# hungpham2511/toppra

Hardware: NVIDIA H100
Metric: paths/sec (7-DOF, 200 gridpoints, vel+accel) (higher is better)
Workload: dtype f64

## Files before the change

toppra_b200/csrc/tb_scan.cu:

```cuda
#include <limits.h>

#include "tb_common.cuh"
#include "tb_scan_common.cuh"

namespace tb {
namespace {

__device__ __forceinline__ uint32_t smem_u32(const void *p) { return (uint32_t)__cvta_generic_to_shared(p); }

__device__ __forceinline__ void mbar_init(uint64_t *bar, unsigned count) {
  asm volatile("mbarrier.init.shared::cta.b64 [%0], %1;" ::"r"(smem_u32(bar)), "r"(count) : "memory");
}
__device__ __forceinline__ void mbar_expect_tx_s(uint32_t bar, unsigned bytes) {
  asm volatile("mbarrier.arrive.expect_tx.shared::cta.b64 _, [%0], %1;" ::"r"(bar), "r"(bytes) : "memory");
}
__device__ __forceinline__ void bulk_g2s_s(uint32_t dst, const void *src, unsigned bytes, uint32_t bar) {
  asm volatile("cp.async.bulk.shared::cluster.global.mbarrier::complete_tx::bytes [%0], [%1], %2, [%3];" ::"r"(dst),
               "l"(src), "r"(bytes), "r"(bar)
               : "memory");
}
__device__ __forceinline__ void mbar_wait_s(const uint32_t addr, unsigned parity) {
  uint32_t ok;
  do {
    asm volatile(
        "{\n"
        " .reg .pred p;\n"
        " mbarrier.try_wait.parity.shared::cta.b64 p, [%1], %2;\n"
        " selp.u32 %0, 1, 0, p;\n"
        "}\n"
        : "=r"(ok)
        : "r"(addr), "r"(parity)
        : "memory");
    if (!ok) __nanosleep(64);
  } while (!ok);
}

__device__ __forceinline__ double warp_min(double v) {
  const int hi = __double2hiint(v), lo = __double2loint(v);
  const int m = hi >> 31;
  const unsigned khi = (unsigned)(hi ^ (m | (int)0x80000000)), klo = (unsigned)(lo ^ m);
  const unsigned mh = __reduce_min_sync(FULL, khi);
  const unsigned ml = __reduce_min_sync(FULL, khi == mh ? klo : 0xffffffffu);
  const int m2 = ((int)~mh) >> 31;
  return __hiloint2double((int)(mh ^ (unsigned)(m2 | (int)0x80000000)), (int)(ml ^ (unsigned)m2));
}
__device__ __forceinline__ double warp_max(double v) {
  const int hi = __double2hiint(v), lo = __double2loint(v);
  const int m = hi >> 31;
  const unsigned khi = (unsigned)(hi ^ (m | (int)0x80000000)), klo = (unsigned)(lo ^ m);
  const unsigned mh = __reduce_max_sync(FULL, khi);
  const unsigned ml = __reduce_max_sync(FULL, khi == mh ? klo : 0u);
  const int m2 = ((int)~mh) >> 31;
  return __hiloint2double((int)(mh ^ (unsigned)(m2 | (int)0x80000000)), (int)(ml ^ (unsigned)m2));
}

constexpr int SCAN_NBUF = 4;

__device__ __forceinline__ void project_item(const bool part, const double aj, const double bj, const double cj,
                                             const double dt0, const double dt1, const double z0, const double z1,
                                             double &thi, double &tlo, bool &bad) {
  const double denom = dt0 * aj + dt1 * bj;
  const double num = cj + z1 * bj + z0 * aj;
  const bool up = part && (denom > LP_TINY), dn = part && (denom < -LP_TINY);
  const double t = -num / ((up || dn) ? denom : 1.0);
  thi = (up && t < LP_INF) ? t : LP_INF;
  tlo = (dn && t > -LP_INF) ? t : -LP_INF;
  bad = bad || (part && !(up || dn) && (num > LP_SMALL));
}

__device__ __forceinline__ void box_row(const int m, const double low0, const double high0, const double low1,
                                        const double high1, double &aj, double &bj, double &cj) {
  aj = __hiloint2double((m == 0) ? (int)0xBFF00000 : ((m == 1) ? 0x3FF00000 : 0), 0);
  bj = __hiloint2double((m == 2) ? (int)0xBFF00000 : ((m == 3) ? 0x3FF00000 : 0), 0);
  cj = (m < 2) ? ((m == 0) ? low0 : -high0) : ((m == 2) ? low1 : -high1);
}

template <int RPL, bool PERM, bool SKIP>
__device__ __forceinline__ bool lp2d_impl(const double v0, const double v1, const double (&a)[RPL],
                                          const double (&b)[RPL], const double (&c)[RPL], const int nC,
                                          const double low0, const double high0, const double low1,
                                          const double high1, int &ac0, int &ac1, double &out_u, double &out_x,
                                          const int lane, int &n_resolve) {
  double p0 = (v0 > LP_TINY) ? high0 : low0;
  double p1 = (v1 > LP_TINY) ? high1 : low1;
  int nac0 = (v0 > LP_TINY) ? -2 : -1;
  int nac1 = (v1 > LP_TINY) ? -4 : -3;
  constexpr bool valid = PERM;
  int pos[RPL];
#pragma unroll
  for (int s = 0; s < RPL; ++s) {
    const int r = lane + 32 * s;
// ... 153 lines not shown
    if (__any_sync(FULL, bad || cross)) return false;
    if (tstar == (pick_min ? -LP_INF : LP_INF)) return false;
    int mykey = INT_MAX;
#pragma unroll
    for (int s = 0; s < RPL; ++s) mykey = ((pick_min ? tlo[s] : thi[s]) == tstar) ? min(mykey, key[s]) : mykey;
    if (!box_inline) mykey = ((pick_min ? xlo_t : xhi_t) == tstar) ? min(mykey, BOXBASE + lane) : mykey;
    const int akey = __reduce_min_sync(FULL, mykey);
    nac1 = (akey >= BOXBASE) ? (-1 - (akey - BOXBASE)) : pos_row(akey, valid, ac0, ac1);
    p0 = z0 + tstar * dt0;
    p1 = z1 + tstar * dt1;
  }
  ac0 = nac0;
  ac1 = nac1;
  out_u = p0;
  out_x = p1;
  return true;
}

template <int RPL, bool SKIP = false>
__device__ __forceinline__ bool lp2d_warp(const double v0, const double v1, const double (&a)[RPL],
                                          const double (&b)[RPL], const double (&c)[RPL], const int nC,
                                          const double low0, const double high0, const double low1,
                                          const double high1, int &ac0, int &ac1, double &out_u, double &out_x,
                                          const int lane, int &n_resolve) {
  if (low0 > high0 || low1 > high1) return false;
  const bool valid = ac0 >= 0 && ac0 < nC && ac1 >= 0 && ac1 < nC && ac0 != ac1;
  if (valid)
    return lp2d_impl<RPL, true, SKIP>(v0, v1, a, b, c, nC, low0, high0, low1, high1, ac0, ac1, out_u, out_x, lane,
                                       n_resolve);
  return lp2d_impl<RPL, false, SKIP>(v0, v1, a, b, c, nC, low0, high0, low1, high1, ac0, ac1, out_u, out_x, lane,
                                     n_resolve);
}

template <int RPL>
__device__ __forceinline__ bool lp1d_fixed_x_warp(const double v0, const double x, const double (&a)[RPL],
                                                  const double (&b)[RPL], const double (&c)[RPL],
                                                  const double low0, const double high0, double &out_u) {
  double my_hi = high0, my_lo = low0;
#pragma unroll
  for (int s = 0; s < RPL; ++s) {
    const double bxc = b[s] * x + c[s];
    const bool up = a[s] > LP_TINY, dn = a[s] < -LP_TINY;
    const double den = (up || dn) ? a[s] : 1.0;
    const bool zn = (bxc == 0.0);
    const double q = -opaque(zn ? 1.0 : bxc) / den;
    const double t = zn ? (-bxc) * den : q;
    my_hi = (up && t < my_hi) ? t : my_hi;
    my_lo = (dn && t > my_lo) ? t : my_lo;
  }
  const bool pick_min = (fabs(v0) < LP_TINY) || (v0 < 0);
  const double red = warp_min(pick_min ? -my_lo : my_hi);
  const double ustar = pick_min ? -red : red;
  if (__any_sync(FULL, pick_min ? (my_hi < ustar) : (my_lo > ustar))) return false;
  out_u = ustar;
  return true;
}

template <int RPL>
__device__ __forceinline__ void load_rows(const double *rec, const int R, const int nC, const int lane,
                                          double (&a)[RPL], double (&b)[RPL], double (&c)[RPL]) {
#pragma unroll
  for (int s = 0; s < RPL; ++s) {
    const int r = lane + 32 * s;
    const bool in = (r >= 2) && (r < nC);
    const int j = in ? r - 2 : 0;
    const double va = rec[j], vb = rec[R + j], vc = rec[2 * R + j];
    a[s] = in ? va : 0.0;
    b[s] = in ? vb : 0.0;
    c[s] = in ? vc : -1.0;
  }
}

template <int RPL>
__device__ __forceinline__ void set_xnext_rows(const int lane, const double delta, const double xn_min,
                                               const double xn_max, double (&a)[RPL], double (&b)[RPL],
                                               double (&c)[RPL]) {
  const bool xr = lane < 2, first = lane == 0;
  const double sgn = first ? -1.0 : 1.0;
  a[0] = xr ? sgn * (2 * delta) : a[0];
  b[0] = xr ? sgn : b[0];
  c[0] = xr ? (first ? xn_min : -xn_max) : c[0];
}

template <int RPL, int MINB, bool FAST, int CFLAGS = -1, bool FUSED = false, bool UB = false>
__global__ void __launch_bounds__(32, MINB)
scan_kernel(const double *__restrict__ records, const int W, const int R, const double *__restrict__ grid,
            const int grid_shared, const int B, const int G, const double *__restrict__ sd_start,
            const double *__restrict__ sd_end, const double *__restrict__ sd_end_hi, const int flags_arg,
            double *__restrict__ Kout, double *__restrict__ sdout, double *__restrict__ uout,
            int *__restrict__ status, int *__restrict__ fail_stage, int *__restrict__ counters,
            const int *__restrict__ glen, const VelAccSrc src) {
  static_assert(!FUSED || RPL == 1, "the fused row source holds one row per lane");
  static_assert(!(FUSED && UB), "velocity + acceleration problems have no u-bound");
  extern __shared__ __align__(16) unsigned char smem_raw[];
  int lane;
  asm volatile("mov.u32 %0, %%tid.x;" : "=r"(lane));
  const long path = blockIdx.x;
  if (path >= B) return;
  double *bufs = reinterpret_cast<double *>(smem_raw);
  uint64_t *bars = reinterpret_cast<uint64_t *>(smem_raw + (size_t)(FUSED ? 1 : SCAN_NBUF) * W * sizeof(double));
  const int Gp = (CFLAGS < 0 && glen) ? min(max(glen[path], 1), G) : G;
  const int N = Gp - 1, nC = R + 2;
  const unsigned rec_bytes = (unsigned)(W * sizeof(double));
  const void *volatile *sptr = reinterpret_cast<const void *volatile *>(
      smem_raw + (size_t)(FUSED ? 1 : SCAN_NBUF) * W * sizeof(double) + SCAN_NBUF * sizeof(uint64_t));
  if (lane == 0) {
    sptr[0] = FUSED ? static_cast<const void *>(src.xbound + (size_t)path * G * 2)
                    : static_cast<const void *>(records + (size_t)path * G * W);
    sptr[1] = grid + (grid_shared ? 0 : (size_t)path * G);
    sptr[2] = Kout + (size_t)path * G * 2;
  }
  const double *dco = bufs, *sx = bufs + (FUSED ? src.nseg * src.dof * 6 : 0);
  bool f_isrow = false, f_neg = false;
  int f_second = 0, f_k = 0, f_seg = 0;
  double f_c = -1.0;
  if constexpr (FUSED) {
    const int nseg = src.nseg, dof = src.dof;
    const double *cpp = src.ppoly + (size_t)path * 4 * nseg * dof;
    const double *xb = src.breaks + (src.breaks_shared ? 0 : (size_t)path * (nseg + 1));
    double *dco_w = bufs, *sx_w = bufs + nseg * dof * 6;
    for (int q = lane; q < nseg * dof; q += 32) {
      const double c0 = cpp[q], c1 = cpp[nseg * dof + q], c2 = cpp[2 * nseg * dof + q];
      const double d0 = c0 * 3.0, d1 = c1 * 2.0, d2 = c2 * 1.0;
      double *o = dco_w + q * 6;
      o[0] = d0; o[1] = d1; o[2] = d2; o[3] = d0 * 2.0; o[4] = d1 * 1.0; o[5] = 0.0;
    }
    for (int q = lane; q <= nseg; q += 32) sx_w[q] = xb[q];
    const int rr = lane - 2;
    f_isrow = (lane >= 2) && (lane < nC);
    const int blk = f_isrow ? rr / dof : 0;
    f_k = f_isrow ? rr - blk * dof : 0;
    f_neg = (blk & 1) != 0;
    f_second = blk >> 1;
    const double *al = src.alim + (src.lim_shared ? 0 : (size_t)path * dof * 2);
    f_c = f_isrow ? (f_neg ? (0.0 - (-al[f_k * 2 + 0])) : (0.0 - al[f_k * 2 + 1])) : -1.0;
  }
  __syncwarp();
  auto rec_path = [&]() { return static_cast<const double *>(sptr[0]); };
  auto gp = [&]() { return static_cast<const double *>(sptr[1]); };
  auto Kp = [&]() { return static_cast<double *>(const_cast<void *>(sptr[2])); };
  const int flags = (CFLAGS >= 0) ? CFLAGS : flags_arg;
  const bool backward_only = (flags & 1) != 0;
  const bool forward_only = (flags & 16) != 0;
  constexpr bool fast_lower = FAST;
  const bool sd_mode = (flags & 4) != 0;
  const bool sd_slow = (flags & 8) != 0;
  double *sdp = backward_only ? nullptr : sdout + (size_t)path * G;
  double *up = backward_only ? nullptr : uout + (size_t)path * (G > 1 ? G - 1 : 0);

  if (!FUSED && lane == 0) {
#pragma unroll
    for (int q = 0; q < SCAN_NBUF; ++q) mbar_init(&bars[q], 1);
    asm volatile("fence.mbarrier_init.release.cluster;" ::: "memory");
    asm volatile("fence.proxy.async.shared::cta;" ::: "memory");
  }
  __syncwarp();

  unsigned n_issued = 0, n_waited = 0;
  const uint32_t bufs_s = smem_u32(bufs), bars_s = smem_u32(bars);
  auto issue = [&](int stage) {
    if (!FUSED && lane == 0) {
      const unsigned q = n_issued % SCAN_NBUF;
      mbar_expect_tx_s(bars_s + q * 8u, rec_bytes);
      bulk_g2s_s(bufs_s + q * rec_bytes, rec_path() + (size_t)stage * W, rec_bytes, bars_s + q * 8u);
    }
    ++n_issued;
  };
  auto acquire = [&]() -> const double * {
    const unsigned q = n_waited % SCAN_NBUF;
    if (!FUSED) mbar_wait_s(bars_s + q * 8u, (n_waited / SCAN_NBUF) & 1);
    ++n_waited;
    return bufs + (size_t)q * W;
  };
  constexpr int AHEAD = SCAN_NBUF - 1;
  auto fused_row = [&](const double s0, const double s1, const bool down, const double delta, double &ra, double &rb,
                       double &rc) {
    const double s = f_second ? s1 : s0;
    if (down) { while (f_seg > 0 && s < sx[f_seg]) --f_seg; }
    else { while (f_seg < src.nseg - 1 && s >= sx[f_seg + 1]) ++f_seg; }
    const double ds = s - sx[f_seg];
    const double2 *o = reinterpret_cast<const double2 *>(dco + (f_seg * src.dof + f_k) * 6);
    const double2 o01 = o[0], o23 = o[1], o45 = o[2];
    double z = ds;
    double v1 = 0.0 + o23.x;
    v1 = v1 + o01.y * z;
    z = z * ds;
    v1 = v1 + o01.x * z;
    double v2 = 0.0 + o45.x;
    v2 = v2 + o23.y * ds;
    const double va = f_second ? (v1 + (2 * delta) * v2) : v1;
    ra = f_isrow ? (f_neg ? -va : va) : 0.0;
    rb = f_isrow ? (f_neg ? -v2 : v2) : 0.0;
    rc = f_c;
  };

  constexpr bool COUNT = (CFLAGS < 0);
  int n_resolve = 0, n_retry = 0, n_fast = 0;
  double a[RPL], b[RPL], c[RPL];

  const double sde = sd_end ? sd_end[path] : 0.0;
  const double sds = sd_start ? sd_start[path] : 0.0;
  const double sdeh = sd_end_hi ? sd_end_hi[path] : sde;
  double kn0 = sde * sde, kn1 = sdeh * sdeh;
  if (lane == 0 && !forward_only) { double *kq = Kp(); kq[2 * N] = kn0; kq[2 * N + 1] = kn1; }
  int st = TB_STATUS_OK, fstage = -1;
  int up0 = 0, up1 = 0, dn0 = 0, dn1 = 0;
  if (forward_only) {
    st = status[path];
    fstage = fail_stage ? fail_stage[path] : -1;
    { const double *kq = Kp(); kn0 = kq[0]; kn1 = kq[1]; }
  }
  for (int q = 0; !FUSED && !forward_only && q < AHEAD && N - 1 - q >= 0; ++q) issue(N - 1 - q);
  double2 xb_ahead = make_double2(0.0, 0.0);
  if constexpr (FUSED) {
    f_seg = src.nseg - 1;
    if (!forward_only && N > 0) xb_ahead = reinterpret_cast<const double2 *>(rec_path())[N - 1];
  }
  for (int i = forward_only ? -1 : N - 1; i >= 0; --i) {
    const double *gq = gp();
    const double g0 = gq[i], g1 = gq[i + 1];
    const double delta = g1 - g0;
    double xlo, xhi;
    double ulo = VAR_MIN, uhi = VAR_MAX;
    if constexpr (FUSED) {
      fused_row(g0, g1, true, delta, a[0], b[0], c[0]);
      xlo = xb_ahead.x;
      xhi = xb_ahead.y;
      if (i > 0) xb_ahead = reinterpret_cast<const double2 *>(rec_path())[i - 1];
    } else {
      const double *rec = acquire();
      load_rows<RPL>(rec, R, nC, lane, a, b, c);
      xlo = rec[3 * R];
      xhi = rec[3 * R + 1];
      if constexpr (UB) { ulo = rec[3 * R + 2]; uhi = rec[3 * R + 3]; }
      __syncwarp();
      if (i - AHEAD >= 0) issue(i - AHEAD);
    }
    set_xnext_rows<RPL>(lane, delta, kn0, kn1, a, b, c);
    double uu, xx;
    const bool ok_hi = lp2d_warp<RPL, true>(-1e-9, 1.0, a, b, c, nC, ulo, uhi, xlo, xhi, dn0, dn1, uu, xx, lane,
                                      n_resolve);
    const double x_upper = ok_hi ? xx : __longlong_as_double(0x7ff8000000000000LL);
    bool ok_lo;
    double x_lower;
    double ufeas;
    if (fast_lower && xlo <= xhi && lp1d_fixed_x_warp<RPL>(1.0, xlo, a, b, c, ulo, uhi, ufeas)) {
      ok_lo = true;
      x_lower = xlo;
      ++n_fast;
    } else {
        ok_lo = lp2d_warp<RPL, true>(1e-9, -1.0, a, b, c, nC, ulo, uhi, xlo, xhi, up0, up1, uu, xx, lane,
                                   n_resolve);
      x_lower = ok_lo ? xx : __longlong_as_double(0x7ff8000000000000LL);
    }
    if (x_lower < 0) x_lower = 0;
    if (lane == 0) { double *kq = Kp(); kq[2 * i] = x_lower; kq[2 * i + 1] = x_upper; }
    if (!(ok_hi && ok_lo)) {
      st = TB_STATUS_FAIL_UNCONTROLLABLE;
      fstage = i;
      { double *kq = Kp(); for (int j = lane; j < 2 * i; j += 32) kq[j] = 0.0; }
      break;
    }
    kn0 = x_lower;
    kn1 = x_upper;
  }
  if (COUNT && counters && lane == 0 && !forward_only) {
    const int nb = (st == TB_STATUS_OK) ? N : N - fstage;
    counters[path * 4 + 0] = 2 * nb - n_fast;
    counters[path * 4 + 1] = n_fast;
  }
  while (n_waited < n_issued) (void)acquire();
  __syncwarp();

  const double nan_d = __longlong_as_double(0x7ff8000000000000LL);
  const double x_start = sds * sds;
  if (Gp < G && !forward_only) {
    double *kq = Kp();
    for (int j = 2 * Gp + lane; j < 2 * G; j += 32) kq[j] = nan_d;
  }
  if (backward_only) {
    if (lane == 0) {
      status[path] = st;
      if (fail_stage) fail_stage[path] = fstage;
    }
    return;
  }
  if (st == TB_STATUS_OK) {
    if (x_start + ALG_SMALL < kn0 || kn1 + ALG_SMALL < x_start) { st = TB_STATUS_FAIL_UNCONTROLLABLE; fstage = 0; }
  }
  if (st != TB_STATUS_OK) {
    for (int j = lane; j < Gp; j += 32) sdp[j] = nan_d;
    for (int j = lane; j < N; j += 32) up[j] = nan_d;
  } else {
    double x = x_start;
    if (lane == 0) sdp[0] = x;
    for (int q = 0; !FUSED && q < AHEAD && q < N; ++q) issue(q);
    int i = 0;
    if constexpr (FUSED) f_seg = 0;
    for (; i < N; ++i) {
      const double *gq = gp();
      const double g0 = gq[i], g1 = gq[i + 1];
      const double delta = g1 - g0;
      double f_ulo = VAR_MIN, f_uhi = VAR_MAX;
      if constexpr (FUSED) {
        fused_row(g0, g1, false, delta, a[0], b[0], c[0]);
      } else {
        const double *rec = acquire();
        load_rows<RPL>(rec, R, nC, lane, a, b, c);
        if constexpr (UB) { f_ulo = rec[3 * R + 2]; f_uhi = rec[3 * R + 3]; }
        __syncwarp();
        if (i + AHEAD < N) issue(i + AHEAD);
      }
      const double *kq = Kp();
      const double k0 = kq[2 * (i + 1)], k1 = kq[2 * (i + 1) + 1];
      set_xnext_rows<RPL>(lane, delta, k0, k1, a, b, c);
      int tries = 0;
      bool ok;
      double uopt = 0.0;
      while (true) {
          ok = lp1d_fixed_x_warp<RPL>(sd_slow ? -(2 * delta) : -(-2 * delta), x, a, b, c, f_ulo, f_uhi, uopt);
        if (ok || sd_mode || tries >= MAX_TRIES) break;
        x = py_max(x - ALG_TINY, 0.999 * x);
        ++tries;
        ++n_retry;
      }
      if (!ok) {
        st = TB_STATUS_ERR_UNKNOWN;
        fstage = i;
        if (lane == 0) sdp[i] = x;
        for (int j = i + 1 + lane; j < Gp; j += 32) sdp[j] = nan_d;
        for (int j = i + lane; j < N; j += 32) up[j] = sd_mode ? nan_d : 0.0;
        break;
      }
      double x_next = x + 2 * delta * uopt;
      if (sd_mode) {
        x_next = py_min(k1, py_max(k0, x_next - ALG_SMALL));
      } else {
        x_next = py_max(x_next - ALG_TINY, 0.9999 * x_next);
        x_next = py_min(k1, py_max(k0, x_next));
      }
      if (lane == 0) {
        up[i] = uopt;
        if (tries) sdp[i] = x;
        sdp[i + 1] = x_next;
      }
      x = x_next;
    }
    while (n_waited < n_issued) (void)acquire();
    __syncwarp();
    if (!sd_mode)
      for (int j = lane; j < Gp; j += 32) sdp[j] = sqrt(sdp[j]);
  }
  if (Gp < G) {
    for (int j = Gp + lane; j < G; j += 32) sdp[j] = nan_d;
    for (int j = max(Gp - 1, 0) + lane; j < G - 1; j += 32) up[j] = nan_d;
  }
  if (lane == 0) {
    status[path] = st;
    if (fail_stage) fail_stage[path] = fstage;
    if (COUNT && counters) {
      const int n_fwd_stages = (st == TB_STATUS_OK) ? N : ((st == TB_STATUS_ERR_UNKNOWN) ? fstage + 1 : -1);
      if (forward_only) { counters[path * 4 + 0] = 0; counters[path * 4 + 1] = 0; }
      if (n_fwd_stages >= 0) counters[path * 4 + 1] += n_fwd_stages + n_retry;
      counters[path * 4 + 2] = n_resolve;
      counters[path * 4 + 3] = n_retry;
    }
  }
}

__device__ __forceinline__ long warp_path() { return (long)blockIdx.x + (int)(threadIdx.x >> 5); }

template <int RPL>
__global__ void __launch_bounds__(32)
feasible_kernel(const double *__restrict__ records, const int W, const int R, const double *__restrict__ grid,
                const int grid_shared, const int B, const int G, const int ub, double *__restrict__ Xout) {
  const int lane = threadIdx.x & 31;
  const long path = warp_path();
  if (path >= B) return;
  const int N = G - 1, nC = R + 2;
  const double *rec_path = records + (size_t)path * G * W;
  const double *gp = grid + (grid_shared ? 0 : (size_t)path * G);
  double *Xp = Xout + (size_t)path * G * 2;
  double a[RPL], b[RPL], c[RPL];
  int up0 = 0, up1 = 0, dn0 = 0, dn1 = 0, n_resolve = 0;
  const double nan_d = __longlong_as_double(0x7ff8000000000000LL);
  for (int i = 0; i <= N; ++i) {
    const double *rec = rec_path + (size_t)i * W;
    load_rows<RPL>(rec, R, nC, lane, a, b, c);
    const double xlo = fmax(rec[3 * R], -CVXPY_MAXX), xhi = fmin(rec[3 * R + 1], CVXPY_MAXX);
    const double ulo = ub ? rec[3 * R + 2] : VAR_MIN, uhi = ub ? rec[3 * R + 3] : VAR_MAX;
    if (i < N) {
      const double delta = gp[i + 1] - gp[i];
      set_xnext_rows<RPL>(lane, delta, -CVXPY_MAXX, CVXPY_MAXX, a, b, c);
    }
    double uu, xx;
    const bool ok0 = lp2d_warp<RPL>(-1e-9, -1.0, a, b, c, nC, ulo, uhi, xlo, xhi, up0, up1, uu, xx, lane,
                                    n_resolve);
// ... 105 lines not shown
    l0 = x_lower;
    l1 = x_upper;
  }
  if (lane == 0 && fail_stage) fail_stage[path] = fs;
}

template <int RPL>
__global__ void __launch_bounds__(32)
lp2d_batch_kernel(const double *__restrict__ v, const double *__restrict__ a, const double *__restrict__ b,
                  const double *__restrict__ c, const double *__restrict__ low, const double *__restrict__ high,
                  const int *__restrict__ active_in, const int B, const int n, int *__restrict__ result,
                  double *__restrict__ optval, double *__restrict__ optvar, int *__restrict__ active_out) {
  const int lane = threadIdx.x & 31;
  const long p = warp_path();
  if (p >= B) return;
  double ra[RPL], rb[RPL], rc[RPL];
#pragma unroll
  for (int s = 0; s < RPL; ++s) {
    const int r = lane + 32 * s;
    if (r < n) { ra[s] = a[p * n + r]; rb[s] = b[p * n + r]; rc[s] = c[p * n + r]; }
    else { ra[s] = 0.0; rb[s] = 0.0; rc[s] = -1.0; }
  }
  int ac0 = active_in ? active_in[p * 2] : 0, ac1 = active_in ? active_in[p * 2 + 1] : 0;
  int n_resolve = 0;
  double uu = 0.0, xx = 0.0;
  const double v0 = v[p * 3], v1 = v[p * 3 + 1], v2 = v[p * 3 + 2];
  const bool ok = lp2d_warp<RPL>(v0, v1, ra, rb, rc, n, low[p * 2], high[p * 2], low[p * 2 + 1], high[p * 2 + 1], ac0,
                                 ac1, uu, xx, lane, n_resolve);
  if (lane == 0) {
    result[p] = ok ? 1 : 0;
    const double nan_d = __longlong_as_double(0x7ff8000000000000LL);
    optvar[p * 2] = ok ? uu : nan_d;
    optvar[p * 2 + 1] = ok ? xx : nan_d;
    optval[p] = ok ? (uu * v0 + xx * v1 + v2) : nan_d;
    active_out[p * 2] = ac0;
    active_out[p * 2 + 1] = ac1;
  }
}

__global__ void lp1d_batch_kernel(const double *__restrict__ v, const double *__restrict__ a,
                                  const double *__restrict__ b, const double *__restrict__ low,
                                  const double *__restrict__ high, const int B, const int n,
                                  int *__restrict__ result, double *__restrict__ optval,
                                  double *__restrict__ optvar, int *__restrict__ active_out) {
  const int warp = threadIdx.x >> 5, lane = threadIdx.x & 31;
  const long p = (long)blockIdx.x * (blockDim.x >> 5) + warp;
  if (p >= B) return;
  double my_hi = high[p], my_lo = low[p];
  int hi_idx = INT_MAX, lo_idx = INT_MAX;
  for (int r = lane; r < n; r += 32) {
    const double ar = a[p * n + r], br = b[p * n + r];
    if (ar > LP_TINY) {
      const double cx = -br / ar;
      if (cx < my_hi) { my_hi = cx; hi_idx = r; }
    } else if (ar < -LP_TINY) {
      const double cx = -br / ar;
      if (cx > my_lo) { my_lo = cx; lo_idx = r; }
    }
  }
  const double cur_max = warp_min(my_hi), cur_min = warp_max(my_lo);
  int hk = (hi_idx != INT_MAX && my_hi == cur_max) ? hi_idx : INT_MAX;
  int lk = (lo_idx != INT_MAX && my_lo == cur_min) ? lo_idx : INT_MAX;
  hk = __reduce_min_sync(FULL, hk);
  lk = __reduce_min_sync(FULL, lk);
  if (lane == 0) {
    const double nan_d = __longlong_as_double(0x7ff8000000000000LL);
    const double v0 = v[p * 2], v1 = v[p * 2 + 1];
    if (cur_min > cur_max) {
      result[p] = 0; optval[p] = nan_d; optvar[p] = nan_d; active_out[p] = 0;
    } else if (fabs(v0) < LP_TINY || v0 < 0) {
      result[p] = 1; optvar[p] = cur_min; optval[p] = v0 * cur_min + v1; active_out[p] = (lk == INT_MAX) ? -1 : lk;
    } else {
      result[p] = 1; optvar[p] = cur_max; optval[p] = v0 * cur_max + v1; active_out[p] = (hk == INT_MAX) ? -2 : hk;
    }
  }
}

constexpr int SCAN_WARPS_PER_SM = 32;
constexpr int SCAN_RPL2_WARPS_PER_SM = 24;
constexpr int SCAN_FUSED_WARPS_PER_SM = 28;

using ScanKernel = decltype(&scan_kernel<1, SCAN_WARPS_PER_SM, false>);

template <int MINB, bool FUSED>
ScanKernel scan_build(const int flags, const bool counters_or_glen) {
  const bool fast = (flags & TB_SCAN_FAST_LOWER) != 0;
  const int mode = flags & (TB_SCAN_BACKWARD_ONLY | TB_SCAN_SD_FORWARD | TB_SCAN_SD_SLOW | TB_SCAN_FORWARD_ONLY);
  if (!counters_or_glen) {
    if (mode == 0) return fast ? scan_kernel<1, MINB, true, 0, FUSED> : scan_kernel<1, MINB, false, 0, FUSED>;
    if (mode == TB_SCAN_BACKWARD_ONLY)
      return fast ? scan_kernel<1, MINB, true, TB_SCAN_BACKWARD_ONLY, FUSED>
                  : scan_kernel<1, MINB, false, TB_SCAN_BACKWARD_ONLY, FUSED>;
    if (mode == TB_SCAN_FORWARD_ONLY)
      return fast ? scan_kernel<1, MINB, true, TB_SCAN_FORWARD_ONLY, FUSED>
                  : scan_kernel<1, MINB, false, TB_SCAN_FORWARD_ONLY, FUSED>;
  }
  return fast ? scan_kernel<1, MINB, true, -1, FUSED> : scan_kernel<1, MINB, false, -1, FUSED>;
}

template <int RPL>
int launch_scan(const double *records, int W, int R, const double *grid, int grid_shared, int B, int G,
                const double *sd_start, const double *sd_end, const double *sd_end_hi, int flags, double *K,
                double *sd, double *u, int *status, int *fail_stage, int *counters, const int *glen,
                cudaStream_t stream) {
  const size_t smem = (size_t)SCAN_NBUF * W * sizeof(double) + SCAN_NBUF * sizeof(uint64_t) + 4 * sizeof(void *);
  const bool fast = (flags & TB_SCAN_FAST_LOWER) != 0;
  ScanKernel kern;
  if constexpr (RPL == 1) {
    kern = scan_build<SCAN_WARPS_PER_SM, false>(flags, counters || glen);
  } else {
    kern = fast ? scan_kernel<RPL, 1, true> : scan_kernel<RPL, 1, false>;
  }
  if constexpr (RPL == 2) {
    if (!fast && !counters) kern = scan_kernel<RPL, SCAN_RPL2_WARPS_PER_SM, false>;
  }
  if (flags & TB_SCAN_UBOUND)
    kern = scan_kernel<RPL, 1, false, -1, false, true>;
  if (smem > 48 * 1024) {
    cudaError_t e = cudaFuncSetAttribute(kern, cudaFuncAttributeMaxDynamicSharedMemorySize, (int)smem);
    if (e != cudaSuccess) { set_error("tb_scan: cudaFuncSetAttribute: %s", cudaGetErrorString(e)); return (int)e; }
  }
  kern<<<B, 32, smem, stream>>>(records, W, R, grid, grid_shared, B, G, sd_start, sd_end, sd_end_hi, flags, K, sd, u,
                                status, fail_stage, counters, glen, VelAccSrc{});
  return check_launch("tb_scan");
}

template <int MINB>
int launch_scan_velacc_occ(const VelAccSrc &src, int W, int R, const double *grid, int grid_shared, int B, int G,
                           const double *sd_start, const double *sd_end, const double *sd_end_hi, int flags, double *K,
                           double *sd, double *u, int *status, int *fail_stage, int *counters, const int *glen,
                           cudaStream_t stream) {
  const size_t smem = (size_t)W * sizeof(double) + SCAN_NBUF * sizeof(uint64_t) + 4 * sizeof(void *);
  const ScanKernel kern = scan_build<MINB, true>(flags, counters || glen);
  kern<<<B, 32, smem, stream>>>(nullptr, W, R, grid, grid_shared, B, G, sd_start, sd_end, sd_end_hi, flags, K, sd, u,
                                status, fail_stage, counters, glen, src);
  return check_launch("tb_scan_velacc");
}

int launch_scan_velacc(const VelAccSrc &src, int W, int R, const double *grid, int grid_shared, int B, int G,
                       const double *sd_start, const double *sd_end, const double *sd_end_hi, int flags, double *K,
                       double *sd, double *u, int *status, int *fail_stage, int *counters, const int *glen,
                       cudaStream_t stream) {
  const auto launch = ((long)B <= (long)num_sms() * SCAN_FUSED_WARPS_PER_SM)
                          ? launch_scan_velacc_occ<SCAN_FUSED_WARPS_PER_SM>
                          : launch_scan_velacc_occ<SCAN_WARPS_PER_SM>;
  const int mode = flags & (TB_SCAN_BACKWARD_ONLY | TB_SCAN_SD_FORWARD | TB_SCAN_SD_SLOW | TB_SCAN_FORWARD_ONLY);
  if ((mode == 0 || mode == TB_SCAN_FORWARD_ONLY) && !counters && !glen && forward_threads_supported(src.dof, B)) {
    if (mode == 0) {
      const int bflags = (flags & TB_SCAN_FAST_LOWER) | TB_SCAN_BACKWARD_ONLY;
      const int rc = launch(src, W, R, grid, grid_shared, B, G, sd_start, sd_end, sd_end_hi, bflags, K, nullptr, nullptr,
                            status, fail_stage, nullptr, nullptr, stream);
      if (rc) return rc;
    }
    return launch_forward_threads(src, R == 4 * src.dof, grid, grid_shared, B, G, sd_start, K, sd, u, status, fail_stage, stream);
  }
  return launch(src, W, R, grid, grid_shared, B, G, sd_start, sd_end, sd_end_hi, flags, K, sd, u, status, fail_stage,
                counters, glen, stream);
}

template <int RPL>
int launch_feasible(const double *records, int W, int R, const double *grid, int grid_shared, int B, int G,
                    int ub, double *X, cudaStream_t stream) {
  feasible_kernel<RPL><<<B, 32, 0, stream>>>(records, W, R, grid, grid_shared, B, G, ub, X);
  return check_launch("tb_feasible_sets");
}

template <int RPL>
int launch_reachable(const double *records, int W, int R, const double *grid, int grid_shared, int B, int G,
                     const double *sdmin, const double *sdmax, int flags, double *X, double *L, int *fail_stage,
                     cudaStream_t stream) {
  if (flags & TB_SCAN_UBOUND)
    reachable_kernel<RPL, true><<<B, 32, 0, stream>>>(records, W, R, grid, grid_shared, B, G, sdmin, sdmax, X, L, fail_stage);
  else
    reachable_kernel<RPL, false><<<B, 32, 0, stream>>>(records, W, R, grid, grid_shared, B, G, sdmin, sdmax, X, L, fail_stage);
  return check_launch("tb_reachable_sets");
}

int check_scan_args(const char *fn, const void *records, int W, int R, const void *grid, int B, int G) {
  if (!records || !grid || B <= 0 || G <= 0 || R < 0) { set_error("%s: bad argument", fn); return TB_ERR_ARG; }
  if (R > MAX_ROWS) { set_error("%s: R=%d > %d rows", fn, R, MAX_ROWS); return TB_ERR_UNSUPPORTED; }
  if (W < 3 * R + 2 || (W & 1)) { set_error("%s: record stride W=%d must be even and >= 3R+2", fn, W); return TB_ERR_ALIGN; }
  if (((uintptr_t)records & 15) != 0) { set_error("%s: records not 16-byte aligned", fn); return TB_ERR_ALIGN; }
  return 0;
}

}
}

extern "C" int tb_scan_ragged(const double *records, int W, int R, const double *grid, int grid_shared, int B, int G,
                              const int *glen, const double *sd_start, const double *sd_end, const double *sd_end_hi,
                              int flags, double *K, double *sd, double *u, int *status, int *fail_stage, int *counters,
                              void *stream) {
  using namespace tb;
  int rc = check_scan_args("tb_scan", records, W, R, grid, B, G);
  if (rc) return rc;
  if ((flags & TB_SCAN_UBOUND) && W < 3 * R + 4) { set_error("tb_scan: TB_SCAN_UBOUND needs records of W >= 3R+4 doubles"); return TB_ERR_ARG; }
  if ((flags & TB_SCAN_UBOUND) && (flags & TB_SCAN_FAST_LOWER)) { set_error("tb_scan: TB_SCAN_UBOUND excludes TB_SCAN_FAST_LOWER"); return TB_ERR_UNSUPPORTED; }
  if (glen && grid_shared) { set_error("tb_scan: ragged batches (glen) need per-path grids [B][G]"); return TB_ERR_ARG; }
  const bool backward_only = (flags & TB_SCAN_BACKWARD_ONLY) != 0;
  if (!K || !status || (!backward_only && (!sd || (G > 1 && !u)))) { set_error("tb_scan: null output"); return TB_ERR_ARG; }
  cudaStream_t s = (cudaStream_t)stream;
  const int nC = R + 2;
  if (nC <= 32) return launch_scan<1>(records, W, R, grid, grid_shared, B, G, sd_start, sd_end, sd_end_hi, flags, K, sd, u, status, fail_stage, counters, glen, s);
  if (nC <= 64) return launch_scan<2>(records, W, R, grid, grid_shared, B, G, sd_start, sd_end, sd_end_hi, flags, K, sd, u, status, fail_stage, counters, glen, s);
  if (nC <= 96) return launch_scan<3>(records, W, R, grid, grid_shared, B, G, sd_start, sd_end, sd_end_hi, flags, K, sd, u, status, fail_stage, counters, glen, s);
  return launch_scan<4>(records, W, R, grid, grid_shared, B, G, sd_start, sd_end, sd_end_hi, flags, K, sd, u, status, fail_stage, counters, glen, s);
}

extern "C" int tb_scan_ex(const double *records, int W, int R, const double *grid, int grid_shared, int B, int G,
                          const double *sd_start, const double *sd_end, const double *sd_end_hi, int flags, double *K,
                          double *sd, double *u, int *status, int *fail_stage, int *counters, void *stream) {
  return tb_scan_ragged(records, W, R, grid, grid_shared, B, G, nullptr, sd_start, sd_end, sd_end_hi, flags, K, sd, u,
                        status, fail_stage, counters, stream);
}

extern "C" int tb_scan_velacc_ragged(const double *ppoly, const double *breaks, int breaks_shared, int nseg, int dof,
// ... 112 lines not shown
```

Baseline: 2.689 million.

## Stage K and x-bounds in shared memory for fused vel+acc scan

```diff
diff --git a/toppra_b200/csrc/tb_scan.cu b/toppra_b200/csrc/tb_scan.cu
--- a/toppra_b200/csrc/tb_scan.cu
+++ b/toppra_b200/csrc/tb_scan.cu
@@ -7,6 +7,10 @@
 namespace {
 
 __device__ __forceinline__ uint32_t smem_u32(const void *p) { return (uint32_t)__cvta_generic_to_shared(p); }
+__device__ __forceinline__ unsigned opaque_u32(unsigned v) {
+  asm volatile("" : "+r"(v));
+  return v;
+}
 
 __device__ __forceinline__ void mbar_init(uint64_t *bar, unsigned count) {
   asm volatile("mbarrier.init.shared::cta.b64 [%0], %1;" ::"r"(smem_u32(bar)), "r"(count) : "memory");
@@ -326,7 +330,7 @@
   c[0] = xr ? (first ? xn_min : -xn_max) : c[0];
 }
 
-template <int RPL, int MINB, bool FAST, int CFLAGS = -1, bool FUSED = false, bool UB = false>
+template <int RPL, int MINB, bool FAST, int CFLAGS = -1, bool FUSED = false, bool UB = false, bool SMEM_K = false>
 __global__ void __launch_bounds__(32, MINB)
 scan_kernel(const double *__restrict__ records, const int W, const int R, const double *__restrict__ grid,
             const int grid_shared, const int B, const int G, const double *__restrict__ sd_start,
@@ -336,6 +340,7 @@
             const int *__restrict__ glen, const VelAccSrc src) {
   static_assert(!FUSED || RPL == 1, "the fused row source holds one row per lane");
   static_assert(!(FUSED && UB), "velocity + acceleration problems have no u-bound");
+  static_assert(!SMEM_K || FUSED, "only the fused scan stages K in shared memory");
   extern __shared__ __align__(16) unsigned char smem_raw[];
   int lane;
   asm volatile("mov.u32 %0, %%tid.x;" : "=r"(lane));
@@ -343,6 +348,17 @@
   if (path >= B) return;
   double *bufs = reinterpret_cast<double *>(smem_raw);
   uint64_t *bars = reinterpret_cast<uint64_t *>(smem_raw + (size_t)(FUSED ? 1 : SCAN_NBUF) * W * sizeof(double));
+  double *fc_s = reinterpret_cast<double *>(bars + SCAN_NBUF) + 4;
+  double2 *kx = reinterpret_cast<double2 *>(fc_s + 32);
+  if constexpr (SMEM_K) {
+    if (!(((CFLAGS >= 0) ? CFLAGS : flags_arg) & TB_SCAN_FORWARD_ONLY) && lane == 0) {
+      mbar_init(&bars[0], 1);
+      asm volatile("fence.mbarrier_init.release.cluster;" ::: "memory");
+      asm volatile("fence.proxy.async.shared::cta;" ::: "memory");
+      mbar_expect_tx_s(smem_u32(bars), (unsigned)G * 16u);
+      bulk_g2s_s(smem_u32(kx), src.xbound + (size_t)path * G * 2, (unsigned)G * 16u, smem_u32(bars));
+    }
+  }
   const int Gp = (CFLAGS < 0 && glen) ? min(max(glen[path], 1), G) : G;
   const int N = Gp - 1, nC = R + 2;
   const unsigned rec_bytes = (unsigned)(W * sizeof(double));
@@ -355,9 +371,8 @@
     sptr[2] = Kout + (size_t)path * G * 2;
   }
   const double *dco = bufs, *sx = bufs + (FUSED ? src.nseg * src.dof * 6 : 0);
-  bool f_isrow = false, f_neg = false;
-  int f_second = 0, f_k = 0, f_seg = 0;
-  double f_c = -1.0;
+  unsigned f_row = 0;
+  int f_seg = 0;
   if constexpr (FUSED) {
     const int nseg = src.nseg, dof = src.dof;
     const double *cpp = src.ppoly + (size_t)path * 4 * nseg * dof;
@@ -371,13 +386,13 @@
     }
     for (int q = lane; q <= nseg; q += 32) sx_w[q] = xb[q];
     const int rr = lane - 2;
-    f_isrow = (lane >= 2) && (lane < nC);
+    const bool f_isrow = (lane >= 2) && (lane < nC);
     const int blk = f_isrow ? rr / dof : 0;
-    f_k = f_isrow ? rr - blk * dof : 0;
-    f_neg = (blk & 1) != 0;
-    f_second = blk >> 1;
+    const int f_k = f_isrow ? rr - blk * dof : 0;
+    const bool f_neg = (blk & 1) != 0;
+    f_row = (f_isrow ? 1u : 0u) | (f_neg ? 2u : 0u) | ((blk >> 1) ? 4u : 0u) | ((unsigned)(f_k * 6) << 8);
     const double *al = src.alim + (src.lim_shared ? 0 : (size_t)path * dof * 2);
-    f_c = f_isrow ? (f_neg ? (0.0 - (-al[f_k * 2 + 0])) : (0.0 - al[f_k * 2 + 1])) : -1.0;
+    fc_s[lane] = f_isrow ? (f_neg ? (0.0 - (-al[f_k * 2 + 0])) : (0.0 - al[f_k * 2 + 1])) : -1.0;
   }
   __syncwarp();
   auto rec_path = [&]() { return static_cast<const double *>(sptr[0]); };
@@ -419,11 +434,13 @@
   constexpr int AHEAD = SCAN_NBUF - 1;
   auto fused_row = [&](const double s0, const double s1, const bool down, const double delta, double &ra, double &rb,
                        double &rc) {
+    const unsigned fr = opaque_u32(f_row);
+    const bool f_isrow = (fr & 1u) != 0, f_neg = (fr & 2u) != 0, f_second = (fr & 4u) != 0;
     const double s = f_second ? s1 : s0;
     if (down) { while (f_seg > 0 && s < sx[f_seg]) --f_seg; }
     else { while (f_seg < src.nseg - 1 && s >= sx[f_seg + 1]) ++f_seg; }
     const double ds = s - sx[f_seg];
-    const double2 *o = reinterpret_cast<const double2 *>(dco + (f_seg * src.dof + f_k) * 6);
+    const double2 *o = reinterpret_cast<const double2 *>(dco + f_seg * src.dof * 6 + (int)(fr >> 8));
     const double2 o01 = o[0], o23 = o[1], o45 = o[2];
     double z = ds;
     double v1 = 0.0 + o23.x;
@@ -435,7 +452,7 @@
     const double va = f_second ? (v1 + (2 * delta) * v2) : v1;
     ra = f_isrow ? (f_neg ? -va : va) : 0.0;
     rb = f_isrow ? (f_neg ? -v2 : v2) : 0.0;
-    rc = f_c;
+    rc = static_cast<const volatile double *>(fc_s)[lane];
   };
 
   constexpr bool COUNT = (CFLAGS < 0);
@@ -446,19 +463,31 @@
   const double sds = sd_start ? sd_start[path] : 0.0;
   const double sdeh = sd_end_hi ? sd_end_hi[path] : sde;
   double kn0 = sde * sde, kn1 = sdeh * sdeh;
-  if (lane == 0 && !forward_only) { double *kq = Kp(); kq[2 * N] = kn0; kq[2 * N + 1] = kn1; }
+  if constexpr (SMEM_K) {
+    if (!forward_only) {
+      mbar_wait_s(bars_s, 0);
+      if (lane == 0) kx[N] = make_double2(kn0, kn1);
+    }
+  } else {
+    if (lane == 0 && !forward_only) { double *kq = Kp(); kq[2 * N] = kn0; kq[2 * N + 1] = kn1; }
+  }
   int st = TB_STATUS_OK, fstage = -1;
   int up0 = 0, up1 = 0, dn0 = 0, dn1 = 0;
   if (forward_only) {
     st = status[path];
     fstage = fail_stage ? fail_stage[path] : -1;
     { const double *kq = Kp(); kn0 = kq[0]; kn1 = kq[1]; }
+    if constexpr (SMEM_K) {
+      const double *kq = Kp();
+      double *kxd = reinterpret_cast<double *>(kx);
+      for (int j = lane; j < 2 * G; j += 32) kxd[j] = kq[j];
+    }
   }
   for (int q = 0; !FUSED && !forward_only && q < AHEAD && N - 1 - q >= 0; ++q) issue(N - 1 - q);
   double2 xb_ahead = make_double2(0.0, 0.0);
   if constexpr (FUSED) {
     f_seg = src.nseg - 1;
-    if (!forward_only && N > 0) xb_ahead = reinterpret_cast<const double2 *>(rec_path())[N - 1];
+    if (!SMEM_K && !forward_only && N > 0) xb_ahead = reinterpret_cast<const double2 *>(rec_path())[N - 1];
   }
   for (int i = forward_only ? -1 : N - 1; i >= 0; --i) {
     const double *gq = gp();
@@ -468,9 +497,15 @@
     double ulo = VAR_MIN, uhi = VAR_MAX;
     if constexpr (FUSED) {
       fused_row(g0, g1, true, delta, a[0], b[0], c[0]);
-      xlo = xb_ahead.x;
-      xhi = xb_ahead.y;
-      if (i > 0) xb_ahead = reinterpret_cast<const double2 *>(rec_path())[i - 1];
+      if constexpr (SMEM_K) {
+        const double2 xb = kx[i];
+        xlo = xb.x;
+        xhi = xb.y;
+      } else {
+        xlo = xb_ahead.x;
+        xhi = xb_ahead.y;
+        if (i > 0) xb_ahead = reinterpret_cast<const double2 *>(rec_path())[i - 1];
+      }
     } else {
       const double *rec = acquire();
       load_rows<RPL>(rec, R, nC, lane, a, b, c);
@@ -493,16 +528,20 @@
       x_lower = xlo;
       ++n_fast;
     } else {
-        ok_lo = lp2d_warp<RPL, true>(1e-9, -1.0, a, b, c, nC, ulo, uhi, xlo, xhi, up0, up1, uu, xx, lane,
-                                   n_resolve);
+      ok_lo = lp2d_warp<RPL, true>(1e-9, -1.0, a, b, c, nC, ulo, uhi, xlo, xhi, up0, up1, uu, xx, lane, n_resolve);
       x_lower = ok_lo ? xx : __longlong_as_double(0x7ff8000000000000LL);
     }
     if (x_lower < 0) x_lower = 0;
-    if (lane == 0) { double *kq = Kp(); kq[2 * i] = x_lower; kq[2 * i + 1] = x_upper; }
+    if constexpr (SMEM_K) {
+      __syncwarp();
+      if (lane == 0) kx[i] = make_double2(x_lower, x_upper);
+    } else {
+      if (lane == 0) { double *kq = Kp(); kq[2 * i] = x_lower; kq[2 * i + 1] = x_upper; }
+    }
     if (!(ok_hi && ok_lo)) {
       st = TB_STATUS_FAIL_UNCONTROLLABLE;
       fstage = i;
-      { double *kq = Kp(); for (int j = lane; j < 2 * i; j += 32) kq[j] = 0.0; }
+      { double *kq = SMEM_K ? reinterpret_cast<double *>(kx) : Kp(); for (int j = lane; j < 2 * i; j += 32) kq[j] = 0.0; }
       break;
     }
     kn0 = x_lower;
@@ -519,8 +558,14 @@
   const double nan_d = __longlong_as_double(0x7ff8000000000000LL);
   const double x_start = sds * sds;
   if (Gp < G && !forward_only) {
+    double *kq = SMEM_K ? reinterpret_cast<double *>(kx) : Kp();
+    for (int j = 2 * Gp + lane; j < 2 * G; j += 32) kq[j] = nan_d;
+  }
+  if (SMEM_K && !forward_only) {
+    __syncwarp();
     double *kq = Kp();
-    for (int j = 2 * Gp + lane; j < 2 * G; j += 32) kq[j] = nan_d;
+    const double *kxd = reinterpret_cast<const double *>(kx);
+    for (int j = lane; j < 2 * G; j += 32) kq[j] = kxd[j];
   }
   if (backward_only) {
     if (lane == 0) {
@@ -555,8 +600,16 @@
         __syncwarp();
         if (i + AHEAD < N) issue(i + AHEAD);
       }
-      const double *kq = Kp();
-      const double k0 = kq[2 * (i + 1)], k1 = kq[2 * (i + 1) + 1];
+      double k0, k1;
+      if constexpr (SMEM_K) {
+        const double2 kk = kx[i + 1];
+        k0 = kk.x;
+        k1 = kk.y;
+      } else {
+        const double *kq = Kp();
+        k0 = kq[2 * (i + 1)];
+        k1 = kq[2 * (i + 1) + 1];
+      }
       set_xnext_rows<RPL>(lane, delta, k0, k1, a, b, c);
       int tries = 0;
       bool ok;
@@ -828,20 +881,32 @@
 
 using ScanKernel = decltype(&scan_kernel<1, SCAN_WARPS_PER_SM, false>);
 
-template <int MINB, bool FUSED>
+template <int MINB, bool FUSED, bool SMEM_K = false>
 ScanKernel scan_build(const int flags, const bool counters_or_glen) {
   const bool fast = (flags & TB_SCAN_FAST_LOWER) != 0;
   const int mode = flags & (TB_SCAN_BACKWARD_ONLY | TB_SCAN_SD_FORWARD | TB_SCAN_SD_SLOW | TB_SCAN_FORWARD_ONLY);
   if (!counters_or_glen) {
-    if (mode == 0) return fast ? scan_kernel<1, MINB, true, 0, FUSED> : scan_kernel<1, MINB, false, 0, FUSED>;
+    if (mode == 0)
+      return fast ? scan_kernel<1, MINB, true, 0, FUSED, false, SMEM_K> : scan_kernel<1, MINB, false, 0, FUSED, false, SMEM_K>;
     if (mode == TB_SCAN_BACKWARD_ONLY)
-      return fast ? scan_kernel<1, MINB, true, TB_SCAN_BACKWARD_ONLY, FUSED>
-                  : scan_kernel<1, MINB, false, TB_SCAN_BACKWARD_ONLY, FUSED>;
+      return fast ? scan_kernel<1, MINB, true, TB_SCAN_BACKWARD_ONLY, FUSED, false, SMEM_K>
+                  : scan_kernel<1, MINB, false, TB_SCAN_BACKWARD_ONLY, FUSED, false, SMEM_K>;
     if (mode == TB_SCAN_FORWARD_ONLY)
-      return fast ? scan_kernel<1, MINB, true, TB_SCAN_FORWARD_ONLY, FUSED>
-                  : scan_kernel<1, MINB, false, TB_SCAN_FORWARD_ONLY, FUSED>;
-  }
-  return fast ? scan_kernel<1, MINB, true, -1, FUSED> : scan_kernel<1, MINB, false, -1, FUSED>;
+      return fast ? scan_kernel<1, MINB, true, TB_SCAN_FORWARD_ONLY, FUSED, false, SMEM_K>
+                  : scan_kernel<1, MINB, false, TB_SCAN_FORWARD_ONLY, FUSED, false, SMEM_K>;
+  }
+  return fast ? scan_kernel<1, MINB, true, -1, FUSED, false, SMEM_K> : scan_kernel<1, MINB, false, -1, FUSED, false, SMEM_K>;
+}
+
+bool smem_fits(const size_t smem, const int ctas, int *carveout) {
+  int dev = 0, per_sm = 0, reserved = 0;
+  if (cudaGetDevice(&dev) != cudaSuccess ||
+      cudaDeviceGetAttribute(&per_sm, cudaDevAttrMaxSharedMemoryPerMultiprocessor, dev) != cudaSuccess ||
+      cudaDeviceGetAttribute(&reserved, cudaDevAttrReservedSharedMemoryPerBlock, dev) != cudaSuccess || per_sm <= 0)
+    return false;
+  const size_t need = (size_t)ctas * (((smem + 127) & ~(size_t)127) + (size_t)reserved);
+  *carveout = (int)((100 * need + per_sm - 1) / per_sm);
+  return need <= (size_t)per_sm;
 }
 
 template <int RPL>
@@ -876,8 +941,18 @@
                            const double *sd_start, const double *sd_end, const double *sd_end_hi, int flags, double *K,
                            double *sd, double *u, int *status, int *fail_stage, int *counters, const int *glen,
                            cudaStream_t stream) {
-  const size_t smem = (size_t)W * sizeof(double) + SCAN_NBUF * sizeof(uint64_t) + 4 * sizeof(void *);
-  const ScanKernel kern = scan_build<MINB, true>(flags, counters || glen);
+  size_t smem = (size_t)W * sizeof(double) + SCAN_NBUF * sizeof(uint64_t) + 4 * sizeof(void *) + 32 * sizeof(double);
+  const size_t smem_k = smem + (size_t)G * 2 * sizeof(double);
+  int carveout = 0;
+  ScanKernel kern;
+  if (smem_fits(smem_k, MINB, &carveout)) {
+    kern = scan_build<MINB, true, true>(flags, counters || glen);
+    smem = smem_k;
+    cudaError_t e = cudaFuncSetAttribute(kern, cudaFuncAttributePreferredSharedMemoryCarveout, carveout);
+    if (e != cudaSuccess) { set_error("tb_scan_velacc: cudaFuncSetAttribute: %s", cudaGetErrorString(e)); return (int)e; }
+  } else {
+    kern = scan_build<MINB, true>(flags, counters || glen);
+  }
   kern<<<B, 32, smem, stream>>>(nullptr, W, R, grid, grid_shared, B, G, sd_start, sd_end, sd_end_hi, flags, K, sd, u,
                                 status, fail_stage, counters, glen, src);
   return check_launch("tb_scan_velacc");
```

Result: faster. 2.917 million, median of 6 (+8.5%).
